# dkotfis/Octree-SLAM

Hardware: AMD Instinct MI355X
Metric: SLAM frames/sec (fuse+ICP+raycast) (higher is better)
Workload: dtype u32/f32 (ICP sums exact fixed-point in f64); 1 GPU; cfg3: synthetic 640x480 RGB-D stream, depth-12 SVO, half-edge 4.096 m, bilateral+ICP(19 it)+fuse+raycast(reference mode); parallelism=single GPU, frames_in_map_at_end=300, frames_input=resident in HBM

## Files before the change

octree-slam_amd/csrc/cone_trace.hip:

```cpp
#include <cstdio>
#include <cstdlib>
#include <cstring>
#include <map>
#include <memory>
#include <mutex>
#include <type_traits>
#include <vector>

#include "config.hpp"
#include "cone_trace.hpp"
#include "pool_grid.hpp"
#include "stage_timing.hpp"
#include "workspace.hpp"

namespace svoslam {

__device__ constexpr float kMaxRange = 10.0f;
__device__ constexpr float kStartDist = 0.002f;
constexpr int kMaxSteps = 1 << 20;

__device__ inline int step_lod(float size, float pix_size) {
  const uint32_t ua = f2bits(size), ub = f2bits(pix_size);
  const int ea = (int)((ua >> 23) & 0xFF), eb = (int)((ub >> 23) & 0xFF);
  if (ea == 0 || eb == 0 || ea == 255 || eb == 255 || (int32_t)ua < 0 || (int32_t)ub < 0 || ea - eb > 120 || eb - ea > 120) {
// ... 368 lines not shown
          yb = axis_bits_lds<LDSD>(ty, P.lo[1], P.inv_cell_lds, lds_tab + kLdsStride, ok);
          zb = axis_bits_lds<LDSD>(tz, P.lo[2], P.inv_cell_lds, lds_tab + 2 * kLdsStride, ok);
        }
      }
      if (!ok) {
        xb = axis_bits_chain(tx, P.center[0], P.size, kLdsDepth);
        yb = axis_bits_chain(ty, P.center[1], P.size, kLdsDepth);
        zb = axis_bits_chain(tz, P.center[2], P.size, kLdsDepth);
      }
      asm volatile("" :: "v"(xb), "v"(yb), "v"(zb));
      uint32_t w1 = 0;
      uint32_t oct_l[kLdsDepth - kGridLevel];
#pragma unroll
      for (int q = 0; q < kLdsDepth - kGridLevel; q++) {
        const int sh = kLdsDepth - kGridLevel - 1 - q;
        oct_l[q] = ((xb >> sh) & 1u) | (((yb >> sh) & 1u) << 1) | (((zb >> sh) & 1u) << 2);
        asm volatile("" : "+v"(oct_l[q]));
      }
      if (depth >= kGridLevel) {
        const uint32_t cell = ((zb >> (kLdsDepth - kGridLevel)) << (2 * kGridLevel)) | ((yb >> (kLdsDepth - kGridLevel)) << kGridLevel) |
                              (xb >> (kLdsDepth - kGridLevel));
        uint2 g = g_s;
        if (cell != cell_s) g = *reinterpret_cast<const uint2 *>(reinterpret_cast<const char *>(grid) + (cell << 3));
        w1 = g.y;
        asm volatile("" :: "v"(w1));
        if (!(g.x & kFlag)) {
          depth = (int)g.x;
        } else if (depth > kGridLevel) {
          uint32_t child_idx = g.x & kMask;
          const int lds_end = depth < kLdsDepth ? depth : kLdsDepth;
          bool stopped = false;
#pragma unroll
          for (int q = 0; q < kLdsDepth - kGridLevel; q++) {
            const int l = kGridLevel + 1 + q;
            if (!stopped && l <= lds_end) {
              uint2 nd = nodes[child_idx + oct_l[q]];
              asm volatile("" : "+v"(nd.y));
              w1 = nd.y;
              if (!(nd.x & kFlag)) { depth = l; stopped = true; }
              else child_idx = nd.x & kMask;
            }
          }
          if (!stopped && depth > kLdsDepth) {
            if (ok) walk_deep_chain<LDSD>(nodes, lds_tab, P, tx, ty, tz, xb, yb, zb, child_idx, depth, w1);
            else walk_deep(nodes, table, P, tx, ty, tz, kLdsDepth + 1, child_idx, depth, w1);
          }
        }
      } else if (depth >= 1) {
        const uint32_t cell = pyramid_index<kLdsDepth, kGridLevel>(xb, yb, zb, depth);
        uint2 g = g_s;
        if (cell != cell_s) g = grid[cell];
        w1 = g.y;
        if (!(g.x & kFlag)) depth = (int)g.x;
      } else {
        w1 = octree[1];
      }
      my_levels += (uint32_t)(depth > 0 ? depth : 0);
      oct_val = w1;
      asm volatile("" :: "v"(w1));

      alpha = (int)((oct_val >> 24) - 127u);
      bool retired;
      if (CARRY) {
        const float af = alpha_lut[alpha + 127];
        vx = (vx + f2u8(af * (float)(oct_val & 0xFF))) & 0xFFu;
        vy = (vy + f2u8(af * (float)((oct_val >> 8) & 0xFF))) & 0xFFu;
        vz = (vz + f2u8(af * (float)((oct_val >> 16) & 0xFF))) & 0xFFu;
        retired = !((int)vw + alpha < 127);
        vw = retired ? 255u : ((uint32_t)((int)vw + alpha) & 0xFFu);
      } else {
        retired = !(alpha < 127);
      }
      if (retired) break;
      const float new_dist = (depth >= -100 && depth <= 100) ? ldexpf(P.size, -depth) : P.size / ldexpf(1.0f, depth);
      if (midrange && depth >= -60) {
        const float s = div_rn_midrange_r(ray_len + new_dist, ray_len, inv_len);
        rx *= s; ry *= s; rz *= s;
        ray_len = sqrt_rn_midrange(dot3(rx, ry, rz, rx, ry, rz));
      } else {
        const float s = (ray_len + new_dist) / ray_len;
        rx *= s; ry *= s; rz *= s;
        ray_len = length3(rx, ry, rz);
      }
      asm volatile("" :: "v"(ray_len));
      if (ray_len > kMaxRange) { range_exit = true; break; }
    }
    if (!CARRY) {
      const float af = alpha_lut[alpha + 127];
      vx = f2u8(af * (float)(oct_val & 0xFF));
      vy = f2u8(af * (float)((oct_val >> 8) & 0xFF));
      vz = f2u8(af * (float)((oct_val >> 16) & 0xFF));
      vw = (uint32_t)alpha & 0xFFu;
    }
    uint32_t out = 0;
    if (range_exit) {
      const float sc = 127.0f / (float)vw;
      vx = f2u8((float)vx * sc);
      vy = f2u8((float)vy * sc);
      vz = f2u8((float)vz * sc);
      out = vx | (vy << 8) | (vz << 16) | (255u << 24);
    } else {
      out = vx | (vy << 8) | (vz << 16) | (255u << 24);
    }
    if (P.mode & 0x100) out = my_steps;
    uchar4 o;
    o.x = (unsigned char)(out & 0xFF); o.y = (unsigned char)((out >> 8) & 0xFF);
    o.z = (unsigned char)((out >> 16) & 0xFF); o.w = (unsigned char)(out >> 24);
    pos[idx] = o;
  }
  if (slots) count_steps(slots, counters, my_steps, my_levels, lane);
}


template <int LDSD, int GRID>
__device__ __forceinline__ uint32_t walk_sample(const uint2 *__restrict__ nodes, const uint32_t *__restrict__ octree, const uint2 *__restrict__ grid,
                                             const float *__restrict__ table, const float *lds_tab, const TraceParams &P, float tx, float ty, float tz,
                                             uint32_t xb, uint32_t yb, uint32_t zb, bool ok, int &depth) {
  uint32_t w1 = 0;
  if (depth >= GRID) {
    const uint32_t cell = ((zb >> (LDSD - GRID)) << (2 * GRID)) | ((yb >> (LDSD - GRID)) << GRID) | (xb >> (LDSD - GRID));
    const uint2 g = grid[cell];
    w1 = g.y;
    if (!(g.x & kFlag)) {
      depth = (int)g.x;
    } else if (depth > GRID) {
      uint32_t child_idx = g.x & kMask;
      const int lds_end = depth < LDSD ? depth : LDSD;
      bool stopped = false;
      for (int l = GRID + 1; l <= lds_end; l++) {
        const int sh = LDSD - l;
        const uint32_t oct = ((xb >> sh) & 1u) | (((yb >> sh) & 1u) << 1) | (((zb >> sh) & 1u) << 2);
        const uint2 nd = nodes[child_idx + oct];
        w1 = nd.y;
        if (!(nd.x & kFlag)) { depth = l; stopped = true; break; }
        child_idx = nd.x & kMask;
      }
      if (!stopped && depth > LDSD) {
        if (ok) walk_deep_chain<LDSD>(nodes, lds_tab, P, tx, ty, tz, xb, yb, zb, child_idx, depth, w1);
        else walk_deep(nodes, table, P, tx, ty, tz, LDSD + 1, child_idx, depth, w1);
      }
    }
  } else if (depth >= 1) {
    walk_shallow<LDSD, GRID>(grid, xb, yb, zb, depth, w1);
  } else {
    w1 = octree[1];
  }
  return w1;
}

#ifndef SVO_AHEAD_WAVES
#define SVO_AHEAD_WAVES 6
#endif
struct MarchSample {
  float rx, ry, rz, len;
  float tx, ty, tz;
  int fx, fy, fz;
  int lod;
  uint32_t lod_ok;
  uint2 gq;
  uint32_t e, have_e;
};

template <int THREADS, bool LOD_ALWAYS, int S, int B>
__global__ __launch_bounds__(THREADS, SVO_AHEAD_WAVES) void cone_trace_brick_kernel(uchar4 *__restrict__ pos, const uint32_t *__restrict__ octree,
                                                                   const uint2 *__restrict__ grid, const uint16_t *__restrict__ bricks,
                                                                   const float *__restrict__ table, const float *__restrict__ alpha_lut_g,
                                                                   TraceParams P, unsigned long long *__restrict__ counters,
                                                                   unsigned long long *__restrict__ slots) {
  constexpr int LDSD = 11, GRID = kPoolGridLevel;
  constexpr int kLdsStride = lds_stride(LDSD);
  constexpr int kCells = lds_cells(LDSD);
  constexpr int BL = brick_bits_level(S);
  constexpr int kFine = kCells << S;
  constexpr uint32_t kOrg = brick_window_origin(S);
#ifdef SVO_BRICK_DIAG
  const long long c_entry = clock64();
#endif
  __shared__ float alpha_lut[256];
  __shared__ float lds_tab[3 * kLdsStride + 3 * kCells];
  uint32_t *spread = reinterpret_cast<uint32_t *>(lds_tab + 3 * kLdsStride);
  if (threadIdx.x < 256) alpha_lut[threadIdx.x] = alpha_lut_g[threadIdx.x];
  {
    const float *src = table + 3 * kTabStride;
    for (int i = threadIdx.x; i < 3 * kLdsStride; i += THREADS) lds_tab[i] = src[i];
    for (int i = threadIdx.x; i < kCells; i += THREADS) {
      const uint32_t r = (uint32_t)i;
      spread[i] = (uint32_t)(brick_entry_index(r, 0u, 0u) >> 1);
      spread[kCells + i] = (uint32_t)(brick_entry_index(0u, r, 0u) >> 1);
      spread[2 * kCells + i] = (uint32_t)(brick_entry_index(0u, 0u, r) >> 1);
    }
  }
  __syncthreads();
#ifdef SVO_BRICK_DIAG
  const long long c_tables = clock64();
#endif
  const unsigned wave = threadIdx.x >> 6, lane = threadIdx.x & 63u;
  const int tile_id = P.tile_order ? (int)P.tile_order[blockIdx.x] : (int)blockIdx.x;
  const int tile_y = tile_id / P.xcd_h;
  const int tile_x = tile_id - tile_y * P.xcd_h;
  const int px = tile_x * 32 + (int)(wave & 3u) * 8 + (int)(lane & 7u);
  const int py = P.pair_rows ? P.row_first + (tile_y + (int)(wave >> 2) * P.pair_rows) * 8 + (int)(lane >> 3)
                         : P.row_first + tile_y * (THREADS / 32) + (int)(wave >> 2) * 8 + (int)(lane >> 3);
  uint32_t my_steps = 0, my_levels = 0;
  if (px < P.width && py < P.row_end) {
    const int idx = py * P.width + px;
    const float res_x = (float)P.width, res_y = (float)P.height;
    const float magx = ((float)px - res_x / 2.0f) / 532.57f;
    const float magy = ((float)py - res_y / 2.0f) / 531.54f;
    const float nyx = -P.y_dir[0], nyy = -P.y_dir[1], nyz = -P.y_dir[2];
    const float fx = P.x_dir[1] * nyz - nyy * P.x_dir[2];
    const float fy = P.x_dir[2] * nyx - nyz * P.x_dir[0];
    const float fz = P.x_dir[0] * nyy - nyx * P.x_dir[1];
    const float dx = ((magx * P.x_dir[0]) + (magy * P.y_dir[0])) + fx;
    const float dy = ((magx * P.x_dir[1]) + (magy * P.y_dir[1])) + fy;
    const float dz = ((magx * P.x_dir[2]) + (magy * P.y_dir[2])) + fz;
    const float inv = 1.0f / sqrtf((dx * dx + dy * dy) + dz * dz);
    float rx = kStartDist * (dx * inv), ry = kStartDist * (dy * inv), rz = kStartDist * (dz * inv);
    const uint2 *nodes = reinterpret_cast<const uint2 *>(octree);
    float ray_len = length3(rx, ry, rz);
    const float ts11 = ldexpf(P.size, -LDSD);
    const float ts12 = ldexpf(P.size, -LDSD - 1);
    const float inv_cell_fine = S == 0 ? P.inv_cell_lds : P.inv_cell_lds * 2.0f;
    float tx = 0.0f, ty = 0.0f, tz = 0.0f;
    int lod = 0;
    uint32_t retired = 0;
    uint32_t prev_gx = 0;
    int dprev = 1 << 20;
    bool ray_done = true;
    auto brick_entry = [&](uint32_t x, uint32_t y, uint32_t z) -> uint32_t {
      if (S > 0) {
        x -= kOrg; y -= kOrg; z -= kOrg;
        if ((x | y | z) >= kBrickWindowCells) return 0u;
      }
      const uint32_t d = spread[x] | spread[kCells + y] | spread[2 * kCells + z];
      return *reinterpret_cast<const uint16_t *>(reinterpret_cast<const char *>(bricks) + (((size_t)d << 2) | ((x & 1u) << 1)));
    };
    auto decode = [&](uint32_t e, uint2 gq, int lod_, uint32_t oct12, int &depth, uint32_t &ret) -> bool {
      const int st = S == 0 ? (int)((e & 7u) | 8u) : (int)((0x009DCBA8u >> ((e & 7u) << 2)) & 15u);
      const int depth_b = lod_ < st ? lod_ : st;
      uint32_t bit = (uint32_t)(depth_b - 5);
      constexpr int NLv = brick_node_level(S);
      bool by_brick = (uint32_t)(depth_b - NLv) < 3u;
      if (S > 0) by_brick = by_brick || (st > GRID && st < NLv && depth_b == st);
      if (lod_ >= BL) {
        const bool deep = depth_b == BL && (lod_ == BL || !(e & 8u));
        by_brick = by_brick || deep;
        bit = deep ? 8u + oct12 : bit;
      }
      const uint32_t lv = lod_ < GRID ? (uint32_t)lod_ : (uint32_t)GRID;
      const uint32_t depth_g = gq.x < kFlag ? gq.x : lv;
      const uint32_t top_g = gq.x < kFlag ? 127u : lv;
      const bool by_grid = (uint32_t)lod_ - depth_g <= top_g - depth_g;
      depth = by_brick ? depth_b : (int)depth_g;
      ret = by_brick ? (e >> bit) & 1u : (uint32_t)(gq.y >= 0xFE000000u);
      return by_brick || by_grid;
    };
#ifdef SVO_BRICK_DIAG
    long long c_after_loop = 0;
    uint32_t diag[4] = {0, 0, 0, 0};
    long long clk[3] = {0, 0, 0};
    const long long c_loop = clock64();
#endif
    for (;;) {
#ifdef SVO_BRICK_DIAG
      const long long c0 = clock64();
#endif
      my_steps++;
      tx = P.origin[0] + rx; ty = P.origin[1] + ry; tz = P.origin[2] + rz;
      const float pix_size = ray_len * P.pix_scale;
      int fx_ = (int)((tx - P.lo[0]) * inv_cell_fine), fy_ = (int)((ty - P.lo[1]) * inv_cell_fine), fz_ = (int)((tz - P.lo[2]) * inv_cell_fine);
      fx_ = fx_ < 0 ? 0 : (fx_ > kFine - 1 ? kFine - 1 : fx_);
      fy_ = fy_ < 0 ? 0 : (fy_ > kFine - 1 ? kFine - 1 : fy_);
      fz_ = fz_ < 0 ? 0 : (fz_ > kFine - 1 ? kFine - 1 : fz_);
      const int gx = fx_ >> S, gy = fy_ >> S, gz = fz_ >> S;
      const uint32_t ub = f2bits(pix_size);
      lod = (P.size_exp - (int)(ub >> 23)) + ((ub & 0x7FFFFFu) < P.size_man ? 1 : 0);
      const bool lod_ok = LOD_ALWAYS || ub - P.lod_first <= P.lod_span;
      const bool coarse = (uint32_t)(lod - 1) < (uint32_t)(GRID - 1);
      uint32_t gcell = (((uint32_t)gz >> (LDSD - GRID)) << (2 * GRID)) | (((uint32_t)gy >> (LDSD - GRID)) << GRID) | ((uint32_t)gx >> (LDSD - GRID));
      if (__builtin_expect(__any(coarse), 0)) {
        if (coarse) gcell = pyramid_index<LDSD, GRID>((uint32_t)gx, (uint32_t)gy, (uint32_t)gz, lod);
      }
      const uint2 gq = grid[gcell];
      const bool with_brick = __any((prev_gx & kFlag) != 0u);
      uint32_t e = 0;
      if (with_brick) e = brick_entry((uint32_t)fx_, (uint32_t)fy_, (uint32_t)fz_);
      float inv_len = __builtin_amdgcn_rcpf(ray_len);
      inv_len = fmaf(fmaf(-ray_len, inv_len, 1.0f), inv_len, inv_len);
      const float ax = lds_tab[gx + 1], bx = lds_tab[gx + 2];
      const float ay = lds_tab[kLdsStride + gy + 1], by = lds_tab[kLdsStride + gy + 2];
      const float az = lds_tab[2 * kLdsStride + gz + 1], bz = lds_tab[2 * kLdsStride + gz + 2];
      bool conf = (((int)(ax < tx) & (int)!(bx < tx)) & ((int)(ay < ty) & (int)!(by < ty)) & ((int)(az < tz) & (int)!(bz < tz))) != 0;
#ifdef SVO_BRICK_DIAG
      asm volatile("" :: "v"(conf), "v"(inv_len));
      const long long c1 = clock64();
      asm volatile("s_waitcnt vmcnt(0)" ::: "memory");
      const long long c2 = clock64();
#endif
      prev_gx = coarse ? 0u : gq.x;
      if (!with_brick && __any((gq.x & kFlag) != 0u && lod > GRID && lod_ok)) e = brick_entry((uint32_t)fx_, (uint32_t)fy_, (uint32_t)fz_);
      uint32_t oct12 = 0;
      if (S > 0 || __any(lod >= BL)) {
        float cx = (gx & 1) ? ax : bx, cy = (gy & 1) ? ay : by, cz = (gz & 1) ? az : bz;
        cx += ts11 * ((gx & 1) ? 1.0f : -1.0f);
        cy += ts11 * ((gy & 1) ? 1.0f : -1.0f);
        cz += ts11 * ((gz & 1) ? 1.0f : -1.0f);
        const uint32_t hx = (uint32_t)(tx > cx), hy = (uint32_t)(ty > cy), hz = (uint32_t)(tz > cz);
        if (S == 0) {
          oct12 = hx | (hy << 1) | (hz << 2);
        } else {
          conf = conf && (((hx ^ (uint32_t)fx_) | (hy ^ (uint32_t)fy_) | (hz ^ (uint32_t)fz_)) & 1u) == 0u;
          if (__any(lod >= BL)) {
            cx += ts12 * (hx ? 1.0f : -1.0f);
            cy += ts12 * (hy ? 1.0f : -1.0f);
            cz += ts12 * (hz ? 1.0f : -1.0f);
            oct12 = (uint32_t)(tx > cx) | ((uint32_t)(ty > cy) << 1) | ((uint32_t)(tz > cz) << 2);
          }
        }
      }
      int depth;
      const bool decided = decode(e, gq, lod, oct12, depth, retired);
      float new_dist = ldexpf(P.size, -depth);
      bool full_form = false;
      int depth_raw = depth;
#ifdef SVO_BRICK_DIAG
      if (decided && conf && lod_ok) diag[0]++;
      if (with_brick) diag[2]++;
#endif
      if (__builtin_expect(__any(!(decided && conf && lod_ok)), 0)) {
        if (!(decided && conf && lod_ok)) {
          if (!lod_ok) lod = step_lod(P.size, pix_size);
          bool ok = true;
          uint32_t xb = (uint32_t)gx, yb = (uint32_t)gy, zb = (uint32_t)gz;
          uint32_t e2 = e;
          uint2 g2 = gq;
          if (!conf) {
            xb = axis_bits_lds<LDSD>(tx, P.lo[0], P.inv_cell_lds, lds_tab, ok);
            yb = axis_bits_lds<LDSD>(ty, P.lo[1], P.inv_cell_lds, lds_tab + kLdsStride, ok);
            zb = axis_bits_lds<LDSD>(tz, P.lo[2], P.inv_cell_lds, lds_tab + 2 * kLdsStride, ok);
            if (!ok) {
              xb = axis_bits_chain(tx, P.center[0], P.size, LDSD);
              yb = axis_bits_chain(ty, P.center[1], P.size, LDSD);
              zb = axis_bits_chain(tz, P.center[2], P.size, LDSD);
            }
          }
          if (!conf || !lod_ok) {
            const bool coarse2 = (uint32_t)(lod - 1) < (uint32_t)(GRID - 1);
            g2 = grid[coarse2 ? pyramid_index<LDSD, GRID>(xb, yb, zb, lod)
                              : ((zb >> (LDSD - GRID)) << (2 * GRID)) | ((yb >> (LDSD - GRID)) << GRID) | (xb >> (LDSD - GRID))];
            prev_gx = coarse2 ? 0u : g2.x;
          }
          float cx = lds_tab[(xb & ~1u) + 2u], cy = lds_tab[kLdsStride + (yb & ~1u) + 2u], cz = lds_tab[2 * kLdsStride + (zb & ~1u) + 2u];
          cx += ts11 * ((xb & 1u) ? 1.0f : -1.0f);
          cy += ts11 * ((yb & 1u) ? 1.0f : -1.0f);
          cz += ts11 * ((zb & 1u) ? 1.0f : -1.0f);
          uint32_t oct12r = (uint32_t)(tx > cx) | ((uint32_t)(ty > cy) << 1) | ((uint32_t)(tz > cz) << 2);
          if (S > 0) {
            const uint32_t cxf = (xb << 1) | (oct12r & 1u), cyf = (yb << 1) | ((oct12r >> 1) & 1u), czf = (zb << 1) | (oct12r >> 2);
            if (!conf) e2 = ok ? brick_entry(cxf, cyf, czf) : 0u;
            cx += ts12 * ((oct12r & 1u) ? 1.0f : -1.0f);
            cy += ts12 * ((oct12r & 2u) ? 1.0f : -1.0f);
            cz += ts12 * ((oct12r & 4u) ? 1.0f : -1.0f);
            oct12r = (uint32_t)(tx > cx) | ((uint32_t)(ty > cy) << 1) | ((uint32_t)(tz > cz) << 2);
          } else if (!conf) {
            e2 = ok ? brick_entry(xb, yb, zb) : 0u;
          }
          const bool decided2 = ok && decode(e2, g2, lod, oct12r, depth, retired);
          if (!decided2) {
            depth = lod;
            const uint32_t w = walk_sample<LDSD, GRID>(nodes, octree, grid, table, lds_tab, P, tx, ty, tz, xb, yb, zb, ok, depth);
            retired = (w >> 24) >= 254u ? 1u : 0u;
#ifdef SVO_BRICK_DIAG
            diag[3]++;
#endif
          }
          new_dist = (depth >= -100 && depth <= 100) ? ldexpf(P.size, -depth) : P.size / ldexpf(1.0f, depth);
          full_form = depth < -60;
          depth_raw = depth;
          if (depth < 0) depth = 0;
#ifdef SVO_BRICK_DIAG
          diag[1]++;
#endif
        }
      }
      my_levels += (uint32_t)depth;
#ifdef SVO_BRICK_DIAG
      clk[0] += c1 - c0; clk[1] += c2 - c1;
#endif
      float s = div_rn_midrange_r(ray_len + new_dist, ray_len, inv_len);
      if (__builtin_expect(__any(full_form), 0)) {
        if (full_form) s = (ray_len + new_dist) / ray_len;
      }
      const float nx = rx * s, ny = ry * s, nz = rz * s;
      float nlen = sqrt_rn_midrange(dot3(nx, ny, nz, nx, ny, nz));
      if (__builtin_expect(__any(full_form), 0)) {
        if (full_form) nlen = length3(nx, ny, nz);
      }
#ifdef SVO_BRICK_DIAG
      asm volatile("" :: "v"(nlen));
      clk[2] += clock64() - c2;
#endif
      rx = nx; ry = ny; rz = nz; ray_len = nlen;
      if (B > 0) dprev = depth_raw;
      if (retired != 0u || nlen > kMaxRange || my_steps >= (uint32_t)kMaxSteps) break;
      if (B > 0 && (int)my_steps >= P.spec_from) { ray_done = false; break; }
    }
    if (B > 0 && !ray_done) {
      const char *zero_entry = reinterpret_cast<const char *>(alpha_lut_g + 256);
      auto place = [&](MarchSample &q) {
        q.tx = P.origin[0] + q.rx; q.ty = P.origin[1] + q.ry; q.tz = P.origin[2] + q.rz;
        int fx_ = (int)((q.tx - P.lo[0]) * inv_cell_fine), fy_ = (int)((q.ty - P.lo[1]) * inv_cell_fine), fz_ = (int)((q.tz - P.lo[2]) * inv_cell_fine);
        q.fx = fx_ < 0 ? 0 : (fx_ > kFine - 1 ? kFine - 1 : fx_);
        q.fy = fy_ < 0 ? 0 : (fy_ > kFine - 1 ? kFine - 1 : fy_);
        q.fz = fz_ < 0 ? 0 : (fz_ > kFine - 1 ? kFine - 1 : fz_);
        const uint32_t ub = f2bits(q.len * P.pix_scale);
        q.lod = (P.size_exp - (int)(ub >> 23)) + ((ub & 0x7FFFFFu) < P.size_man ? 1 : 0);
        q.lod_ok = (LOD_ALWAYS || ub - P.lod_first <= P.lod_span) ? 1u : 0u;
      };
      auto request = [&](MarchSample &q, bool with_brick) {
        const uint32_t gx = (uint32_t)(q.fx >> S), gy = (uint32_t)(q.fy >> S), gz = (uint32_t)(q.fz >> S);
        const bool coarse = (uint32_t)(q.lod - 1) < (uint32_t)(GRID - 1);
        uint32_t gcell = ((gz >> (LDSD - GRID)) << (2 * GRID)) | ((gy >> (LDSD - GRID)) << GRID) | (gx >> (LDSD - GRID));
        if (__builtin_expect(__any(coarse), 0)) {
          if (coarse) gcell = pyramid_index<LDSD, GRID>(gx, gy, gz, q.lod);
        }
        q.gq = grid[gcell];
        uint32_t x = (uint32_t)q.fx, y = (uint32_t)q.fy, z = (uint32_t)q.fz;
        bool use = with_brick;
        if (S > 0) {
          x -= kOrg; y -= kOrg; z -= kOrg;
          const bool inwin = (x | y | z) < kBrickWindowCells;
          use = use && inwin;
          x = inwin ? x : 0u; y = inwin ? y : 0u; z = inwin ? z : 0u;
        }
        const uint32_t d = spread[x] | spread[kCells + y] | spread[2 * kCells + z];
        const char *at = use ? reinterpret_cast<const char *>(bricks) + (((size_t)d << 2) | ((x & 1u) << 1)) : zero_entry;
        q.e = *reinterpret_cast<const uint16_t *>(at);
        q.have_e = with_brick ? 1u : 0u;
      };
      auto answer = [&](const MarchSample &q, float &new_dist, bool &full_form, int &lod_used) -> int {
        const int gx = q.fx >> S, gy = q.fy >> S, gz = q.fz >> S;
        const float tx = q.tx, ty = q.ty, tz = q.tz;
        const float ax = lds_tab[gx + 1], bx = lds_tab[gx + 2];
        const float ay = lds_tab[kLdsStride + gy + 1], by = lds_tab[kLdsStride + gy + 2];
        const float az = lds_tab[2 * kLdsStride + gz + 1], bz = lds_tab[2 * kLdsStride + gz + 2];
        bool conf = (((int)(ax < tx) & (int)!(bx < tx)) & ((int)(ay < ty) & (int)!(by < ty)) & ((int)(az < tz) & (int)!(bz < tz))) != 0;
        const int lod = q.lod;
        const bool lod_ok = LOD_ALWAYS || q.lod_ok != 0u;
        const bool coarse = (uint32_t)(lod - 1) < (uint32_t)(GRID - 1);
        const uint2 gq = q.gq;
        const uint32_t e = q.e;
        prev_gx = coarse ? 0u : gq.x;
        const bool need = q.have_e == 0u && (gq.x & kFlag) != 0u && lod > GRID && !coarse;
        uint32_t oct12 = 0;
        if (S > 0 || __any(lod >= BL)) {
          float cx = (gx & 1) ? ax : bx, cy = (gy & 1) ? ay : by, cz = (gz & 1) ? az : bz;
          cx += ts11 * ((gx & 1) ? 1.0f : -1.0f);
          cy += ts11 * ((gy & 1) ? 1.0f : -1.0f);
          cz += ts11 * ((gz & 1) ? 1.0f : -1.0f);
          const uint32_t hx = (uint32_t)(tx > cx), hy = (uint32_t)(ty > cy), hz = (uint32_t)(tz > cz);
          if (S == 0) {
            oct12 = hx | (hy << 1) | (hz << 2);
          } else {
            conf = conf && (((hx ^ (uint32_t)q.fx) | (hy ^ (uint32_t)q.fy) | (hz ^ (uint32_t)q.fz)) & 1u) == 0u;
            if (__any(lod >= BL)) {
              cx += ts12 * (hx ? 1.0f : -1.0f);
              cy += ts12 * (hy ? 1.0f : -1.0f);
              cz += ts12 * (hz ? 1.0f : -1.0f);
              oct12 = (uint32_t)(tx > cx) | ((uint32_t)(ty > cy) << 1) | ((uint32_t)(tz > cz) << 2);
            }
          }
        }
        int depth;
        const bool decided = decode(e, gq, lod, oct12, depth, retired) && !need;
        new_dist = ldexpf(P.size, -depth);
        full_form = false;
        lod_used = lod;
        if (__builtin_expect(__any(!(decided && conf && lod_ok)), 0)) {
          if (!(decided && conf && lod_ok)) {
            int lod2 = lod;
            if (!lod_ok) lod2 = step_lod(P.size, q.len * P.pix_scale);
            lod_used = lod2;
            bool ok = true;
            uint32_t xb = (uint32_t)gx, yb = (uint32_t)gy, zb = (uint32_t)gz;
            uint32_t e2 = e;
            uint2 g2 = gq;
            if (need && conf) e2 = brick_entry((uint32_t)q.fx, (uint32_t)q.fy, (uint32_t)q.fz);
            if (!conf) {
              xb = axis_bits_lds<LDSD>(tx, P.lo[0], P.inv_cell_lds, lds_tab, ok);
              yb = axis_bits_lds<LDSD>(ty, P.lo[1], P.inv_cell_lds, lds_tab + kLdsStride, ok);
              zb = axis_bits_lds<LDSD>(tz, P.lo[2], P.inv_cell_lds, lds_tab + 2 * kLdsStride, ok);
              if (!ok) {
                xb = axis_bits_chain(tx, P.center[0], P.size, LDSD);
                yb = axis_bits_chain(ty, P.center[1], P.size, LDSD);
                zb = axis_bits_chain(tz, P.center[2], P.size, LDSD);
              }
            }
            if (!conf || !lod_ok) {
              const bool coarse2 = (uint32_t)(lod2 - 1) < (uint32_t)(GRID - 1);
              g2 = grid[coarse2 ? pyramid_index<LDSD, GRID>(xb, yb, zb, lod2)
                                : ((zb >> (LDSD - GRID)) << (2 * GRID)) | ((yb >> (LDSD - GRID)) << GRID) | (xb >> (LDSD - GRID))];
              prev_gx = coarse2 ? 0u : g2.x;
            }
            float cx = lds_tab[(xb & ~1u) + 2u], cy = lds_tab[kLdsStride + (yb & ~1u) + 2u], cz = lds_tab[2 * kLdsStride + (zb & ~1u) + 2u];
            cx += ts11 * ((xb & 1u) ? 1.0f : -1.0f);
            cy += ts11 * ((yb & 1u) ? 1.0f : -1.0f);
            cz += ts11 * ((zb & 1u) ? 1.0f : -1.0f);
            uint32_t oct12r = (uint32_t)(tx > cx) | ((uint32_t)(ty > cy) << 1) | ((uint32_t)(tz > cz) << 2);
            if (S > 0) {
              const uint32_t cxf = (xb << 1) | (oct12r & 1u), cyf = (yb << 1) | ((oct12r >> 1) & 1u), czf = (zb << 1) | (oct12r >> 2);
              if (!conf) e2 = ok ? brick_entry(cxf, cyf, czf) : 0u;
              cx += ts12 * ((oct12r & 1u) ? 1.0f : -1.0f);
              cy += ts12 * ((oct12r & 2u) ? 1.0f : -1.0f);
              cz += ts12 * ((oct12r & 4u) ? 1.0f : -1.0f);
              oct12r = (uint32_t)(tx > cx) | ((uint32_t)(ty > cy) << 1) | ((uint32_t)(tz > cz) << 2);
            } else if (!conf) {
              e2 = ok ? brick_entry(xb, yb, zb) : 0u;
            }
            const bool decided2 = ok && decode(e2, g2, lod2, oct12r, depth, retired);
            if (!decided2) {
              depth = lod2;
              const uint32_t w = walk_sample<LDSD, GRID>(nodes, octree, grid, table, lds_tab, P, tx, ty, tz, xb, yb, zb, ok, depth);
              retired = (w >> 24) >= 254u ? 1u : 0u;
            }
            new_dist = (depth >= -100 && depth <= 100) ? ldexpf(P.size, -depth) : P.size / ldexpf(1.0f, depth);
            full_form = depth < -60;
            __builtin_amdgcn_s_waitcnt(0x0F70);
          }
        }
        return depth;
      };
      auto burst = [&](auto n_tag) -> bool {
        constexpr int N = decltype(n_tag)::value;
        MarchSample q[N];
        const bool with_brick = __any((prev_gx & kFlag) != 0u);
        q[0].rx = rx; q[0].ry = ry; q[0].rz = rz; q[0].len = ray_len;
        place(q[0]);
        request(q[0], with_brick);
        if (N > 1) {
          const float nd = ldexpf(P.size, -dprev);
  #pragma unroll
          for (int j = 1; j < N; j++) {
            float il = __builtin_amdgcn_rcpf(q[j - 1].len);
            il = fmaf(fmaf(-q[j - 1].len, il, 1.0f), il, il);
            const float sp = div_rn_midrange_r(q[j - 1].len + nd, q[j - 1].len, il);
            q[j].rx = q[j - 1].rx * sp; q[j].ry = q[j - 1].ry * sp; q[j].rz = q[j - 1].rz * sp;
            q[j].len = sqrt_rn_midrange(dot3(q[j].rx, q[j].ry, q[j].rz, q[j].rx, q[j].ry, q[j].rz));
            place(q[j]);
            request(q[j], with_brick);
          }
        }
        bool done = false, chain = true;
  #pragma unroll
        for (int j = 0; j < N; j++) {
          if (chain) {
            my_steps++;
            float new_dist; bool full_form; int lod_used;
            const int depth = answer(q[j], new_dist, full_form, lod_used);
            my_levels += (uint32_t)(depth > 0 ? depth : 0);
            const bool hit = j + 1 < N && depth == dprev && !full_form;
            dprev = depth;
            if (hit) {
              rx = q[j + 1 < N ? j + 1 : j].rx; ry = q[j + 1 < N ? j + 1 : j].ry; rz = q[j + 1 < N ? j + 1 : j].rz; ray_len = q[j + 1 < N ? j + 1 : j].len;
            } else {
              float il = __builtin_amdgcn_rcpf(q[j].len);
              il = fmaf(fmaf(-q[j].len, il, 1.0f), il, il);
              float s = div_rn_midrange_r(q[j].len + new_dist, q[j].len, il);
              if (full_form) s = (q[j].len + new_dist) / q[j].len;
              rx = q[j].rx * s; ry = q[j].ry * s; rz = q[j].rz * s;
              ray_len = full_form ? length3(rx, ry, rz) : sqrt_rn_midrange(dot3(rx, ry, rz, rx, ry, rz));
            }
            tx = q[j].tx; ty = q[j].ty; tz = q[j].tz; lod = lod_used;
            if (retired != 0u || ray_len > kMaxRange || my_steps >= (uint32_t)kMaxSteps) { done = true; chain = false; }
            else if (!hit) chain = false;
          }
        }
        if (N > 1) __builtin_amdgcn_s_waitcnt(0x0F70);
        return done;
      };
      bool done = false;
      while (!done) done = burst(std::integral_constant<int, (B > 0 ? B : 1)>{});
    }
#ifdef SVO_BRICK_DIAG
    if (counters) {
      if (P.mode & 0x200) {
        c_after_loop = clock64();
        if (lane == 0) { atomicAdd(&counters[2], (unsigned long long)(c_tables - c_entry)); atomicAdd(&counters[3], (unsigned long long)(c_loop - c_tables)); atomicAdd(&counters[4], (unsigned long long)(c_after_loop - c_loop)); }
      } else {
      atomicAdd(&counters[2], (unsigned long long)diag[0]);
      atomicAdd(&counters[3], (unsigned long long)diag[1]);
      }
      uint32_t mx = my_steps;
      for (int o = 32; o > 0; o >>= 1) { const uint32_t v = (uint32_t)__shfl_xor((int)mx, o); mx = v > mx ? v : mx; }
      const unsigned long long top = __ballot(my_steps == mx);
      if (!(P.mode & 0x200) && (int)lane == __ffsll((long long)top) - 1) {
        atomicAdd(&counters[4], (unsigned long long)clk[0]);
        atomicAdd(&counters[5], (unsigned long long)clk[1]);
        atomicAdd(&counters[6], (unsigned long long)clk[2]);
        atomicAdd(&counters[7], (unsigned long long)mx);
      }
    }
#endif
    const bool range_exit = retired == 0u && ray_len > kMaxRange;
    uint32_t w_last;
    {
      bool ok = true;
      uint32_t xb = axis_bits_lds<LDSD>(tx, P.lo[0], P.inv_cell_lds, lds_tab, ok);
      uint32_t yb = axis_bits_lds<LDSD>(ty, P.lo[1], P.inv_cell_lds, lds_tab + kLdsStride, ok);
      uint32_t zb = axis_bits_lds<LDSD>(tz, P.lo[2], P.inv_cell_lds, lds_tab + 2 * kLdsStride, ok);
      if (!ok) {
        xb = axis_bits_chain(tx, P.center[0], P.size, LDSD);
        yb = axis_bits_chain(ty, P.center[1], P.size, LDSD);
        zb = axis_bits_chain(tz, P.center[2], P.size, LDSD);
      }
      int d2 = lod;
      w_last = walk_sample<LDSD, GRID>(nodes, octree, grid, table, lds_tab, P, tx, ty, tz, xb, yb, zb, ok, d2);
    }
    const int alpha = (int)((w_last >> 24) - 127u);
    const float af = alpha_lut[alpha + 127];
    uint32_t vx = f2u8(af * (float)(w_last & 0xFF));
    uint32_t vy = f2u8(af * (float)((w_last >> 8) & 0xFF));
    uint32_t vz = f2u8(af * (float)((w_last >> 16) & 0xFF));
    const uint32_t vw = (uint32_t)alpha & 0xFFu;
    if (range_exit) {
      const float sc = 127.0f / (float)vw;
      vx = f2u8((float)vx * sc);
      vy = f2u8((float)vy * sc);
      vz = f2u8((float)vz * sc);
    }
    uint32_t out = vx | (vy << 8) | (vz << 16) | (255u << 24);
    if (P.mode & 0x100) out = my_steps;
    uchar4 o;
    o.x = (unsigned char)(out & 0xFF); o.y = (unsigned char)((out >> 8) & 0xFF);
    o.z = (unsigned char)((out >> 16) & 0xFF); o.w = (unsigned char)(out >> 24);
    pos[idx] = o;
#ifdef SVO_BRICK_DIAG
    if (counters && (P.mode & 0x200) && lane == 0) { asm volatile("s_waitcnt vmcnt(0)" ::: "memory"); atomicAdd(&counters[5], (unsigned long long)(clock64() - c_after_loop)); }
#endif
  }
  if (P.tile_cost) {
    uint32_t mx = my_steps;
#pragma unroll
    for (int o = 32; o > 0; o >>= 1) { const uint32_t v = (uint32_t)__shfl_xor((int)mx, o); mx = v > mx ? v : mx; }
    if (lane == 0) atomicAdd(&P.tile_cost[tile_id], mx);
  }
  if (slots) count_steps(slots, counters, my_steps, my_levels, lane);
}

#ifndef SVO_AHEAD_BURST
#define SVO_AHEAD_BURST 3
#endif
constexpr int kAheadBurst = SVO_AHEAD_BURST;
constexpr int kBrickMarchStaticLds = 1024 + 4 * (3 * lds_stride(11) + 3 * lds_cells(11));
static int brick_march_lds_pad() {
  static int pad = -1;
  if (pad >= 0) return pad;
  int dev = 0;
  hipDeviceProp_t prop;
  size_t lds = 160 * 1024;
  if (hipGetDevice(&dev) == hipSuccess && hipGetDeviceProperties(&prop, dev) == hipSuccess && prop.maxSharedMemoryPerMultiProcessor > 0)
    lds = (size_t)prop.maxSharedMemoryPerMultiProcessor;
  else
    (void)hipGetLastError();
  long long p = (long long)(lds / 3) + 1 - kBrickMarchStaticLds;
  p = p < 0 ? 0 : ((p + 255) / 256) * 256;
  if (p > 0 && p < 6144 && 2 * (kBrickMarchStaticLds + 6144) <= (long long)lds) p = 6144;
  if (2 * (kBrickMarchStaticLds + p) > (long long)lds || kBrickMarchStaticLds + p > 64 * 1024) p = 0;
  if (getenv("SVOSLAM_DEBUG_LDS")) fprintf(stderr, "svoslam: LDS per CU %zu bytes, brick march pad %lld\n", lds, p);
  pad = (int)p;
  return pad;
}
constexpr int kPairMaxTiles = 1024;
constexpr int kTileOrderMinTiles = 512;
__global__ __launch_bounds__(256) void tile_order_kernel(uint32_t *__restrict__ cost, uint32_t *__restrict__ order, int n) {
  tile_order_block(cost, order, n);
}

static unsigned xcd_mapping(TraceParams &P, int tiles_x, int tiles_y) {
  constexpr int kResidentTiles = 1024;
  if (tiles_x * tiles_y <= kResidentTiles) {
    P.xcd_w = (int)cdiv(tiles_x, 4); P.xcd_h = (int)cdiv(tiles_y, 2);
    return 8u * (unsigned)(P.xcd_w * P.xcd_h);
  }
  P.xcd_w = 0; P.xcd_h = tiles_x;
  return (unsigned)(tiles_x * tiles_y);
}

struct StreamAccel {
  DeviceBuffer buf;
  unsigned long long *count_slots = nullptr;
  bool tables_valid = false;
  const float *tables_at = nullptr;
  int lds_depth = 0;
  float size = 0.0f, center[3] = {0.0f, 0.0f, 0.0f};
  uint32_t *tiles = nullptr;
  int tile_cap = 0, tile_count = 0, tile_w = 0, tile_rows = 0, tile_row_first = 0;
};
static std::mutex g_accel_mu;
static std::map<hipStream_t, std::unique_ptr<StreamAccel>> g_accel;

static int accel_for_stream(hipStream_t stream, StreamAccel **out) {
  std::lock_guard<std::mutex> lock(g_accel_mu);
  auto it = g_accel.find(stream);
  if (it == g_accel.end()) it = g_accel.emplace(stream, std::unique_ptr<StreamAccel>(new StreamAccel())).first;
  *out = it->second.get();
  return SVOSLAM_OK;
}

int cone_trace_release(hipStream_t stream, bool all) {
  if (!all) pool_accel_forget_stream(stream);
  std::lock_guard<std::mutex> lock(g_accel_mu);
  if (all) {
    for (auto &kv : g_accel) { kv.second->buf.release(); if (kv.second->count_slots) (void)hipFree(kv.second->count_slots); if (kv.second->tiles) (void)hipFree(kv.second->tiles); }
    g_accel.clear();
  } else {
    auto it = g_accel.find(stream);
    if (it != g_accel.end()) { it->second->buf.release(); if (it->second->count_slots) (void)hipFree(it->second->count_slots); if (it->second->tiles) (void)hipFree(it->second->tiles); g_accel.erase(it); }
  }
  return SVOSLAM_OK;
}

static void mat4_inverse_host(const float *m, float *out);

int cone_trace_svo(uint8_t *d_pos, int width, int height, int row_first, int rows, float fov, const float view[16],
                   const uint32_t *d_octree, const float center[3], float size, int mode, unsigned long long *d_steps,
                   hipStream_t stream) {
  if (!d_pos || !view || !d_octree || !center || width <= 0 || height <= 0) return SVOSLAM_ERR_INVALID_ARG;
  if (row_first < 0 || rows < 0 || row_first + rows > height) return SVOSLAM_ERR_INVALID_ARG;
  if (rows == 0) return SVOSLAM_OK;
  if ((mode & 0xFF) != SVOSLAM_RENDER_REFERENCE && (mode & 0xFF) != SVOSLAM_RENDER_CARRY) return SVOSLAM_ERR_INVALID_ARG;
// ... 167 lines not shown
```

octree-slam_amd/csrc/config.hip:

```cpp
#include <cstdio>
#include <cstdlib>
#include <cstring>
#include <mutex>

#include "config.hpp"

namespace svoslam {
namespace {
std::mutex g_mu;
bool g_ready = false;
svoslam_config g_cfg;

struct Field { const char *name; int32_t svoslam_config::*member; };
const Field kFields[] = {
    {"march_bricks", &svoslam_config::march_bricks}, {"track_mode", &svoslam_config::track_mode},
    {"track_workers", &svoslam_config::track_workers}, {"track_stream", &svoslam_config::track_stream},
    {"runner_deferred", &svoslam_config::runner_deferred}, {"runner_lead", &svoslam_config::runner_lead},
    {"runner_prio", &svoslam_config::runner_prio}, {"runner_replicas", &svoslam_config::runner_replicas},
    {"runner_timeline", &svoslam_config::runner_timeline}, {"sort_pairs", &svoslam_config::sort_pairs},
    {"graphs", &svoslam_config::graphs}, {"march_ahead", &svoslam_config::march_ahead},
};

bool config_valid(const svoslam_config &c) {
  if (c.runner_replicas != 1 || c.graphs != 0) return false;
  if (c.track_mode < 0 || c.track_mode > 2 || c.track_workers < 0) return false;
  return true;
}

void init_locked() {
  if (g_ready) return;
  memset(&g_cfg, 0, sizeof(g_cfg));
  g_cfg.march_bricks = 1; g_cfg.track_stream = 1; g_cfg.march_ahead = 60;
  g_cfg.runner_deferred = -1; g_cfg.runner_lead = -1; g_cfg.runner_prio = -1; g_cfg.runner_replicas = 1;
  if (const char *e = getenv("SVOSLAM_CONFIG")) {
    const char *p = e;
    while (*p) {
      const char *eq = strchr(p, '='), *end = strchr(p, ',');
      if (!end) end = p + strlen(p);
      bool known = false;
      if (eq && eq < end && eq > p) {
        for (const Field &f : kFields)
          if ((size_t)(eq - p) == strlen(f.name) && strncmp(p, f.name, (size_t)(eq - p)) == 0) {
            known = true;
            svoslam_config trial = g_cfg;
            char *stop = nullptr;
            const long v = strtol(eq + 1, &stop, 10);
            trial.*(f.member) = (int32_t)v;
            if (stop == eq + 1 || stop != end || !config_valid(trial))
              fprintf(stderr, "svoslam: SVOSLAM_CONFIG: value of '%s' rejected (\"%.*s\"); the default stays\n", f.name, (int)(end - p), p);
            else
              g_cfg = trial;
          }
      }
      if (!known && end > p) fprintf(stderr, "svoslam: SVOSLAM_CONFIG: unknown or malformed entry \"%.*s\" ignored\n", (int)(end - p), p);
      p = *end ? end + 1 : end;
    }
  }
  g_ready = true;
}
}

svoslam_config config() {
  std::lock_guard<std::mutex> lock(g_mu);
  init_locked();
  return g_cfg;
}
}

extern "C" {
int svoslam_config_get(svoslam_config *out) {
  if (!out) return SVOSLAM_ERR_INVALID_ARG;
  *out = svoslam::config();
  return SVOSLAM_OK;
}
int svoslam_config_set(const svoslam_config *in) {
  if (!in) return SVOSLAM_ERR_INVALID_ARG;
  if (!svoslam::config_valid(*in)) return SVOSLAM_ERR_INVALID_ARG;
  std::lock_guard<std::mutex> lock(svoslam::g_mu);
  svoslam::init_locked();
  svoslam::g_cfg = *in;
  return SVOSLAM_OK;
}
}
```

Measured before the change: 2703 frames/s.

## Slim speculative march samples and split rare-path handling out of burst loop

```diff
diff --git a/octree-slam_amd/csrc/cone_trace.hip b/octree-slam_amd/csrc/cone_trace.hip
--- a/octree-slam_amd/csrc/cone_trace.hip
+++ b/octree-slam_amd/csrc/cone_trace.hip
@@ -544,13 +544,8 @@
 #define SVO_AHEAD_WAVES 6
 #endif
 struct MarchSample {
-  float rx, ry, rz, len;
-  float tx, ty, tz;
-  int fx, fy, fz;
-  int lod;
-  uint32_t lod_ok;
   uint2 gq;
-  uint32_t e, have_e;
+  uint32_t e;
 };
 
 template <int THREADS, bool LOD_ALWAYS, int S, int B>
@@ -642,7 +637,7 @@
       const uint32_t lv = lod_ < GRID ? (uint32_t)lod_ : (uint32_t)GRID;
       const uint32_t depth_g = gq.x < kFlag ? gq.x : lv;
       const uint32_t top_g = gq.x < kFlag ? 127u : lv;
-      const bool by_grid = (uint32_t)lod_ - depth_g <= top_g - depth_g;
+      const bool by_grid = lod_ >= 1 && (uint32_t)lod_ - depth_g <= top_g - depth_g;
       depth = by_brick ? depth_b : (int)depth_g;
       ret = by_brick ? (e >> bit) & 1u : (uint32_t)(gq.y >= 0xFE000000u);
       return by_brick || by_grid;
@@ -799,25 +794,35 @@
     }
     if (B > 0 && !ray_done) {
       const char *zero_entry = reinterpret_cast<const char *>(alpha_lut_g + 256);
-      auto place = [&](MarchSample &q) {
-        q.tx = P.origin[0] + q.rx; q.ty = P.origin[1] + q.ry; q.tz = P.origin[2] + q.rz;
-        int fx_ = (int)((q.tx - P.lo[0]) * inv_cell_fine), fy_ = (int)((q.ty - P.lo[1]) * inv_cell_fine), fz_ = (int)((q.tz - P.lo[2]) * inv_cell_fine);
-        q.fx = fx_ < 0 ? 0 : (fx_ > kFine - 1 ? kFine - 1 : fx_);
-        q.fy = fy_ < 0 ? 0 : (fy_ > kFine - 1 ? kFine - 1 : fy_);
-        q.fz = fz_ < 0 ? 0 : (fz_ > kFine - 1 ? kFine - 1 : fz_);
-        const uint32_t ub = f2bits(q.len * P.pix_scale);
-        q.lod = (P.size_exp - (int)(ub >> 23)) + ((ub & 0x7FFFFFu) < P.size_man ? 1 : 0);
-        q.lod_ok = (LOD_ALWAYS || ub - P.lod_first <= P.lod_span) ? 1u : 0u;
+      auto place = [&](float sx, float sy, float sz, float sl, float &tx_, float &ty_, float &tz_, uint32_t &fx_, uint32_t &fy_, uint32_t &fz_,
+                       int &lod_, bool &lod_ok_) {
+        tx_ = P.origin[0] + sx; ty_ = P.origin[1] + sy; tz_ = P.origin[2] + sz;
+        int cx = (int)((tx_ - P.lo[0]) * inv_cell_fine), cy = (int)((ty_ - P.lo[1]) * inv_cell_fine), cz = (int)((tz_ - P.lo[2]) * inv_cell_fine);
+        fx_ = (uint32_t)(cx < 0 ? 0 : (cx > kFine - 1 ? kFine - 1 : cx));
+        fy_ = (uint32_t)(cy < 0 ? 0 : (cy > kFine - 1 ? kFine - 1 : cy));
+        fz_ = (uint32_t)(cz < 0 ? 0 : (cz > kFine - 1 ? kFine - 1 : cz));
+        const uint32_t ub = f2bits(sl * P.pix_scale);
+        lod_ = (P.size_exp - (int)(ub >> 23)) + ((ub & 0x7FFFFFu) < P.size_man ? 1 : 0);
+        lod_ok_ = LOD_ALWAYS || ub - P.lod_first <= P.lod_span;
       };
-      auto request = [&](MarchSample &q, bool with_brick) {
-        const uint32_t gx = (uint32_t)(q.fx >> S), gy = (uint32_t)(q.fy >> S), gz = (uint32_t)(q.fz >> S);
-        const bool coarse = (uint32_t)(q.lod - 1) < (uint32_t)(GRID - 1);
+      auto advance = [&](float &sx, float &sy, float &sz, float &sl, float nd, bool full) {
+        float il = __builtin_amdgcn_rcpf(sl);
+        il = fmaf(fmaf(-sl, il, 1.0f), il, il);
+        float s = div_rn_midrange_r(sl + nd, sl, il);
+        if (full) s = (sl + nd) / sl;
+        sx *= s; sy *= s; sz *= s;
+        sl = full ? length3(sx, sy, sz) : sqrt_rn_midrange(dot3(sx, sy, sz, sx, sy, sz));
+      };
+      auto request = [&](uint32_t fx_, uint32_t fy_, uint32_t fz_, int lod_, bool with_brick) -> MarchSample {
+        const uint32_t gx = fx_ >> S, gy = fy_ >> S, gz = fz_ >> S;
+        const bool coarse = (uint32_t)(lod_ - 1) < (uint32_t)(GRID - 1);
         uint32_t gcell = ((gz >> (LDSD - GRID)) << (2 * GRID)) | ((gy >> (LDSD - GRID)) << GRID) | (gx >> (LDSD - GRID));
         if (__builtin_expect(__any(coarse), 0)) {
-          if (coarse) gcell = pyramid_index<LDSD, GRID>(gx, gy, gz, q.lod);
+          if (coarse) gcell = pyramid_index<LDSD, GRID>(gx, gy, gz, lod_);
         }
+        MarchSample q;
         q.gq = grid[gcell];
-        uint32_t x = (uint32_t)q.fx, y = (uint32_t)q.fy, z = (uint32_t)q.fz;
+        uint32_t x = fx_, y = fy_, z = fz_;
         bool use = with_brick;
         if (S > 0) {
           x -= kOrg; y -= kOrg; z -= kOrg;
@@ -828,23 +833,18 @@
         const uint32_t d = spread[x] | spread[kCells + y] | spread[2 * kCells + z];
         const char *at = use ? reinterpret_cast<const char *>(bricks) + (((size_t)d << 2) | ((x & 1u) << 1)) : zero_entry;
         q.e = *reinterpret_cast<const uint16_t *>(at);
-        q.have_e = with_brick ? 1u : 0u;
+        return q;
       };
-      auto answer = [&](const MarchSample &q, float &new_dist, bool &full_form, int &lod_used) -> int {
-        const int gx = q.fx >> S, gy = q.fy >> S, gz = q.fz >> S;
-        const float tx = q.tx, ty = q.ty, tz = q.tz;
+      auto examine = [&](uint32_t &fx_, uint32_t &fy_, uint32_t &fz_, bool &lod_ok, uint32_t &oct12) -> bool {
+        float sx = rx, sy = ry, sz = rz, sl = ray_len;
+        asm volatile("" : "+v"(sx), "+v"(sy), "+v"(sz), "+v"(sl));
+        place(sx, sy, sz, sl, tx, ty, tz, fx_, fy_, fz_, lod, lod_ok);
+        const int gx = (int)(fx_ >> S), gy = (int)(fy_ >> S), gz = (int)(fz_ >> S);
         const float ax = lds_tab[gx + 1], bx = lds_tab[gx + 2];
         const float ay = lds_tab[kLdsStride + gy + 1], by = lds_tab[kLdsStride + gy + 2];
         const float az = lds_tab[2 * kLdsStride + gz + 1], bz = lds_tab[2 * kLdsStride + gz + 2];
         bool conf = (((int)(ax < tx) & (int)!(bx < tx)) & ((int)(ay < ty) & (int)!(by < ty)) & ((int)(az < tz) & (int)!(bz < tz))) != 0;
-        const int lod = q.lod;
-        const bool lod_ok = LOD_ALWAYS || q.lod_ok != 0u;
-        const bool coarse = (uint32_t)(lod - 1) < (uint32_t)(GRID - 1);
-        const uint2 gq = q.gq;
-        const uint32_t e = q.e;
-        prev_gx = coarse ? 0u : gq.x;
-        const bool need = q.have_e == 0u && (gq.x & kFlag) != 0u && lod > GRID && !coarse;
-        uint32_t oct12 = 0;
+        oct12 = 0;
         if (S > 0 || __any(lod >= BL)) {
           float cx = (gx & 1) ? ax : bx, cy = (gy & 1) ? ay : by, cz = (gz & 1) ? az : bz;
           cx += ts11 * ((gx & 1) ? 1.0f : -1.0f);
@@ -854,7 +854,7 @@
           if (S == 0) {
             oct12 = hx | (hy << 1) | (hz << 2);
           } else {
-            conf = conf && (((hx ^ (uint32_t)q.fx) | (hy ^ (uint32_t)q.fy) | (hz ^ (uint32_t)q.fz)) & 1u) == 0u;
+            conf = conf && (((hx ^ fx_) | (hy ^ fy_) | (hz ^ fz_)) & 1u) == 0u;
             if (__any(lod >= BL)) {
               cx += ts12 * (hx ? 1.0f : -1.0f);
               cy += ts12 * (hy ? 1.0f : -1.0f);
@@ -863,111 +863,126 @@
             }
           }
         }
+        return conf;
+      };
+      auto needs_brick = [&](const MarchSample &q, bool with_brick) -> bool {
+        const bool coarse = (uint32_t)(lod - 1) < (uint32_t)(GRID - 1);
+        prev_gx = coarse ? 0u : q.gq.x;
+        return !with_brick && (q.gq.x & kFlag) != 0u && lod > GRID && !coarse;
+      };
+      auto answer = [&](const MarchSample &q, bool with_brick, int &depth) -> bool {
+        uint32_t fx_, fy_, fz_, oct12;
+        bool lod_ok;
+        const bool conf = examine(fx_, fy_, fz_, lod_ok, oct12);
+        const bool need = needs_brick(q, with_brick);
+        return decode(q.e, q.gq, lod, oct12, depth, retired) && !need && conf && lod_ok;
+      };
+      auto answer_rare = [&](const MarchSample &q, bool with_brick, float &new_dist, bool &full_form) -> int {
+        uint32_t fx_, fy_, fz_, oct12;
+        bool lod_ok;
+        const bool conf = examine(fx_, fy_, fz_, lod_ok, oct12);
+        const bool need = needs_brick(q, with_brick);
+        if (!lod_ok) lod = step_lod(P.size, ray_len * P.pix_scale);
+        bool ok = true;
+        uint32_t xb = fx_ >> S, yb = fy_ >> S, zb = fz_ >> S;
+        uint32_t e2 = q.e;
+        uint2 g2 = q.gq;
         int depth;
-        const bool decided = decode(e, gq, lod, oct12, depth, retired) && !need;
-        new_dist = ldexpf(P.size, -depth);
-        full_form = false;
-        lod_used = lod;
-        if (__builtin_expect(__any(!(decided && conf && lod_ok)), 0)) {
-          if (!(decided && conf && lod_ok)) {
-            int lod2 = lod;
-            if (!lod_ok) lod2 = step_lod(P.size, q.len * P.pix_scale);
-            lod_used = lod2;
-            bool ok = true;
-            uint32_t xb = (uint32_t)gx, yb = (uint32_t)gy, zb = (uint32_t)gz;
-            uint32_t e2 = e;
-            uint2 g2 = gq;
-            if (need && conf) e2 = brick_entry((uint32_t)q.fx, (uint32_t)q.fy, (uint32_t)q.fz);
-            if (!conf) {
-              xb = axis_bits_lds<LDSD>(tx, P.lo[0], P.inv_cell_lds, lds_tab, ok);
-              yb = axis_bits_lds<LDSD>(ty, P.lo[1], P.inv_cell_lds, lds_tab + kLdsStride, ok);
-              zb = axis_bits_lds<LDSD>(tz, P.lo[2], P.inv_cell_lds, lds_tab + 2 * kLdsStride, ok);
-              if (!ok) {
-                xb = axis_bits_chain(tx, P.center[0], P.size, LDSD);
-                yb = axis_bits_chain(ty, P.center[1], P.size, LDSD);
-                zb = axis_bits_chain(tz, P.center[2], P.size, LDSD);
-              }
-            }
-            if (!conf || !lod_ok) {
-              const bool coarse2 = (uint32_t)(lod2 - 1) < (uint32_t)(GRID - 1);
-              g2 = grid[coarse2 ? pyramid_index<LDSD, GRID>(xb, yb, zb, lod2)
-                                : ((zb >> (LDSD - GRID)) << (2 * GRID)) | ((yb >> (LDSD - GRID)) << GRID) | (xb >> (LDSD - GRID))];
-              prev_gx = coarse2 ? 0u : g2.x;
-            }
-            float cx = lds_tab[(xb & ~1u) + 2u], cy = lds_tab[kLdsStride + (yb & ~1u) + 2u], cz = lds_tab[2 * kLdsStride + (zb & ~1u) + 2u];
-            cx += ts11 * ((xb & 1u) ? 1.0f : -1.0f);
-            cy += ts11 * ((yb & 1u) ? 1.0f : -1.0f);
-            cz += ts11 * ((zb & 1u) ? 1.0f : -1.0f);
-            uint32_t oct12r = (uint32_t)(tx > cx) | ((uint32_t)(ty > cy) << 1) | ((uint32_t)(tz > cz) << 2);
-            if (S > 0) {
-              const uint32_t cxf = (xb << 1) | (oct12r & 1u), cyf = (yb << 1) | ((oct12r >> 1) & 1u), czf = (zb << 1) | (oct12r >> 2);
-              if (!conf) e2 = ok ? brick_entry(cxf, cyf, czf) : 0u;
-              cx += ts12 * ((oct12r & 1u) ? 1.0f : -1.0f);
-              cy += ts12 * ((oct12r & 2u) ? 1.0f : -1.0f);
-              cz += ts12 * ((oct12r & 4u) ? 1.0f : -1.0f);
-              oct12r = (uint32_t)(tx > cx) | ((uint32_t)(ty > cy) << 1) | ((uint32_t)(tz > cz) << 2);
-            } else if (!conf) {
-              e2 = ok ? brick_entry(xb, yb, zb) : 0u;
-            }
-            const bool decided2 = ok && decode(e2, g2, lod2, oct12r, depth, retired);
-            if (!decided2) {
-              depth = lod2;
-              const uint32_t w = walk_sample<LDSD, GRID>(nodes, octree, grid, table, lds_tab, P, tx, ty, tz, xb, yb, zb, ok, depth);
-              retired = (w >> 24) >= 254u ? 1u : 0u;
-            }
-            new_dist = (depth >= -100 && depth <= 100) ? ldexpf(P.size, -depth) : P.size / ldexpf(1.0f, depth);
-            full_form = depth < -60;
-            __builtin_amdgcn_s_waitcnt(0x0F70);
+        if (need && conf) e2 = brick_entry(fx_, fy_, fz_);
+        if (!conf) {
+          xb = axis_bits_lds<LDSD>(tx, P.lo[0], P.inv_cell_lds, lds_tab, ok);
+          yb = axis_bits_lds<LDSD>(ty, P.lo[1], P.inv_cell_lds, lds_tab + kLdsStride, ok);
+          zb = axis_bits_lds<LDSD>(tz, P.lo[2], P.inv_cell_lds, lds_tab + 2 * kLdsStride, ok);
+          if (!ok) {
+            xb = axis_bits_chain(tx, P.center[0], P.size, LDSD);
+            yb = axis_bits_chain(ty, P.center[1], P.size, LDSD);
+            zb = axis_bits_chain(tz, P.center[2], P.size, LDSD);
           }
         }
+        if (!conf || !lod_ok) {
+          const bool coarse2 = (uint32_t)(lod - 1) < (uint32_t)(GRID - 1);
+          g2 = grid[coarse2 ? pyramid_index<LDSD, GRID>(xb, yb, zb, lod)
+                            : ((zb >> (LDSD - GRID)) << (2 * GRID)) | ((yb >> (LDSD - GRID)) << GRID) | (xb >> (LDSD - GRID))];
+          prev_gx = coarse2 ? 0u : g2.x;
+        }
+        float cx = lds_tab[(xb & ~1u) + 2u], cy = lds_tab[kLdsStride + (yb & ~1u) + 2u], cz = lds_tab[2 * kLdsStride + (zb & ~1u) + 2u];
+        cx += ts11 * ((xb & 1u) ? 1.0f : -1.0f);
+        cy += ts11 * ((yb & 1u) ? 1.0f : -1.0f);
+        cz += ts11 * ((zb & 1u) ? 1.0f : -1.0f);
+        uint32_t oct12r = (uint32_t)(tx > cx) | ((uint32_t)(ty > cy) << 1) | ((uint32_t)(tz > cz) << 2);
+        if (S > 0) {
+          const uint32_t cxf = (xb << 1) | (oct12r & 1u), cyf = (yb << 1) | ((oct12r >> 1) & 1u), czf = (zb << 1) | (oct12r >> 2);
+          if (!conf) e2 = ok ? brick_entry(cxf, cyf, czf) : 0u;
+          cx += ts12 * ((oct12r & 1u) ? 1.0f : -1.0f);
+          cy += ts12 * ((oct12r & 2u) ? 1.0f : -1.0f);
+          cz += ts12 * ((oct12r & 4u) ? 1.0f : -1.0f);
+          oct12r = (uint32_t)(tx > cx) | ((uint32_t)(ty > cy) << 1) | ((uint32_t)(tz > cz) << 2);
+        } else if (!conf) {
+          e2 = ok ? brick_entry(xb, yb, zb) : 0u;
+        }
+        const bool decided2 = ok && decode(e2, g2, lod, oct12r, depth, retired);
+        if (!decided2) {
+          depth = lod;
+          const uint32_t w = walk_sample<LDSD, GRID>(nodes, octree, grid, table, lds_tab, P, tx, ty, tz, xb, yb, zb, ok, depth);
+          retired = (w >> 24) >= 254u ? 1u : 0u;
+        }
+        new_dist = (depth >= -100 && depth <= 100) ? ldexpf(P.size, -depth) : P.size / ldexpf(1.0f, depth);
+        full_form = depth < -60;
         return depth;
+      };
+      auto finish = [&](int depth, float new_dist, bool full_form) -> bool {
+        my_steps++;
+        my_levels += (uint32_t)(depth > 0 ? depth : 0);
+        dprev = depth;
+        advance(rx, ry, rz, ray_len, new_dist, full_form);
+        return retired != 0u || ray_len > kMaxRange || my_steps >= (uint32_t)kMaxSteps;
       };
       auto burst = [&](auto n_tag) -> bool {
         constexpr int N = decltype(n_tag)::value;
         MarchSample q[N];
         const bool with_brick = __any((prev_gx & kFlag) != 0u);
-        q[0].rx = rx; q[0].ry = ry; q[0].rz = rz; q[0].len = ray_len;
-        place(q[0]);
-        request(q[0], with_brick);
-        if (N > 1) {
+        {
           const float nd = ldexpf(P.size, -dprev);
+          float sx = rx, sy = ry, sz = rz, sl = ray_len;
   #pragma unroll
-          for (int j = 1; j < N; j++) {
-            float il = __builtin_amdgcn_rcpf(q[j - 1].len);
-            il = fmaf(fmaf(-q[j - 1].len, il, 1.0f), il, il);
-            const float sp = div_rn_midrange_r(q[j - 1].len + nd, q[j - 1].len, il);
-            q[j].rx = q[j - 1].rx * sp; q[j].ry = q[j - 1].ry * sp; q[j].rz = q[j - 1].rz * sp;
-            q[j].len = sqrt_rn_midrange(dot3(q[j].rx, q[j].ry, q[j].rz, q[j].rx, q[j].ry, q[j].rz));
-            place(q[j]);
-            request(q[j], with_brick);
+          for (int j = 0; j < N; j++) {
+            if (j > 0) advance(sx, sy, sz, sl, nd, false);
+            float px_, py_, pz_;
+            uint32_t fx_, fy_, fz_;
+            int lod_;
+            bool lod_ok_;
+            place(sx, sy, sz, sl, px_, py_, pz_, fx_, fy_, fz_, lod_, lod_ok_);
+            q[j] = request(fx_, fy_, fz_, lod_, with_brick);
           }
         }
-        bool done = false, chain = true;
+        bool done = false, chain = true, rare = false;
   #pragma unroll
         for (int j = 0; j < N; j++) {
           if (chain) {
-            my_steps++;
-            float new_dist; bool full_form; int lod_used;
-            const int depth = answer(q[j], new_dist, full_form, lod_used);
-            my_levels += (uint32_t)(depth > 0 ? depth : 0);
-            const bool hit = j + 1 < N && depth == dprev && !full_form;
-            dprev = depth;
-            if (hit) {
-              rx = q[j + 1 < N ? j + 1 : j].rx; ry = q[j + 1 < N ? j + 1 : j].ry; rz = q[j + 1 < N ? j + 1 : j].rz; ray_len = q[j + 1 < N ? j + 1 : j].len;
+            int depth;
+            if (!answer(q[j], with_brick, depth)) {
+              rare = true; chain = false;
             } else {
-              float il = __builtin_amdgcn_rcpf(q[j].len);
-              il = fmaf(fmaf(-q[j].len, il, 1.0f), il, il);
-              float s = div_rn_midrange_r(q[j].len + new_dist, q[j].len, il);
-              if (full_form) s = (q[j].len + new_dist) / q[j].len;
-              rx = q[j].rx * s; ry = q[j].ry * s; rz = q[j].rz * s;
-              ray_len = full_form ? length3(rx, ry, rz) : sqrt_rn_midrange(dot3(rx, ry, rz, rx, ry, rz));
+              const bool hit = j + 1 < N && depth == dprev;
+              done = finish(depth, ldexpf(P.size, -depth), false);
+              chain = hit && !done;
             }
-            tx = q[j].tx; ty = q[j].ty; tz = q[j].tz; lod = lod_used;
-            if (retired != 0u || ray_len > kMaxRange || my_steps >= (uint32_t)kMaxSteps) { done = true; chain = false; }
-            else if (!hit) chain = false;
           }
         }
         if (N > 1) __builtin_amdgcn_s_waitcnt(0x0F70);
+        if (__builtin_expect(__any(rare), 0)) {
+          if (rare) {
+            float new_dist; bool full_form;
+            float px_, py_, pz_;
+            uint32_t fx_, fy_, fz_;
+            int lod_;
+            bool lod_ok_;
+            place(rx, ry, rz, ray_len, px_, py_, pz_, fx_, fy_, fz_, lod_, lod_ok_);
+            const int depth = answer_rare(request(fx_, fy_, fz_, lod_, true), true, new_dist, full_form);
+            done = finish(depth, new_dist, full_form);
+            __builtin_amdgcn_s_waitcnt(0x0F70);
+          }
+        }
         return done;
       };
       bool done = false;
diff --git a/octree-slam_amd/csrc/config.hip b/octree-slam_amd/csrc/config.hip
--- a/octree-slam_amd/csrc/config.hip
+++ b/octree-slam_amd/csrc/config.hip
@@ -24,6 +24,7 @@
 bool config_valid(const svoslam_config &c) {
   if (c.runner_replicas != 1 || c.graphs != 0) return false;
   if (c.track_mode < 0 || c.track_mode > 2 || c.track_workers < 0) return false;
+  if (c.march_ahead < -1 || c.march_ahead > (1 << 20)) return false;
   return true;
 }
 
```

After: 2558 frames/s (median of 2 runs). 5.4% lower.
